# nnnagle/vq-vae

Measured on AMD Instinct MI355X. Metric: tiles/sec, higher is better.
Workload: dtype bf16

## Files before the change

vq-vae_amd/csrc/film_fused.hip:

```cpp
#include "frl_common.hpp"
#include "frl_host.hpp"
#include "frl_pack.hpp"
#include "frl_reduce.hpp"

typedef bf16x8 frag8;
#define FF_CZ 64
#define FF_HID 32
#define FF_C 12
#define FF_FR_W1 (4 * 2 * 64)
#define FF_FR_W2 64
#define FF_FR_W2T (2 * 64)
#define FF_FR_FWD (FF_FR_W1 + 2 * FF_FR_W2)
#define FF_FR_BWD (FF_FR_FWD + 2 * FF_FR_W2T)
#define FF_SLAB (2 * FF_HID * FF_CZ + 2 * FF_C * FF_HID + 2 * FF_HID + 2 * FF_C)

__device__ __forceinline__ void ff_pack_k4(frag8* __restrict__ dst, const float* __restrict__ W2, int tid, int nthreads) {
  for (int i = tid; i < FF_FR_W2T; i += nthreads) {
    const int lane = i & 63, mb = i >> 6;
    const int r = lane & 15, kc = lane >> 4;
    const int unit = 8 * (r >> 2) + 4 * mb + (r & 3);
    bf16x8 v;
#pragma unroll
    for (int e = 0; e < 8; ++e) {
      const int c = 4 * kc + e;
// ... 38 lines not shown
  }
  bool hit = false;
  frag8* pk = ws_pk;
  if (void* img = frl_pack_cached(jobs, n, off, &hit)) pk = (frag8*)img;
  if (!hit) FRL_LAUNCH(ff_pack_kernel, dim3(8), dim3(256), 0, st, pk, w1g, w1b, w2g, w2b, bwd);
  return pk;
}

__device__ __forceinline__ void ff_hidden(f32x4 (&ha)[4], const LQTile<bf16, 2>& zt, const frag8* __restrict__ w1, const float* __restrict__ tb,
                                          int lane, int kc) {
#pragma unroll
  for (int mb = 0; mb < 4; ++mb) {
    f32x4 acc = *reinterpret_cast<const f32x4*>(tb + 32 * (mb >> 1) + 8 * kc + 4 * (mb & 1));
    acc = mfma16(w1[(mb * 2 + 0) * 64 + lane], zt.f[0], acc);
    ha[mb] = mfma16(w1[(mb * 2 + 1) * 64 + lane], zt.f[1], acc);
  }
}
__device__ __forceinline__ frag8 ff_relu_frag(const f32x4& a, const f32x4& b) {
  return frag8{(bf16)fmaxf(a[0], 0.f), (bf16)fmaxf(a[1], 0.f), (bf16)fmaxf(a[2], 0.f), (bf16)fmaxf(a[3], 0.f),
               (bf16)fmaxf(b[0], 0.f), (bf16)fmaxf(b[1], 0.f), (bf16)fmaxf(b[2], 0.f), (bf16)fmaxf(b[3], 0.f)};
}

__device__ __forceinline__ void ff_tables(float* tb, const float* b1g, const float* b1b, const float* b2g, const float* b2b, int tid, int nthreads) {
  for (int i = tid; i < 96; i += nthreads) {
    float v = 0.f;
    if (i < 32) v = b1g[i];
    else if (i < 64) v = b1b[i - 32];
    else if (i < 80) v = (i - 64) < FF_C ? b2g[i - 64] : 0.f;
    else v = (i - 80) < FF_C ? b2b[i - 80] : 0.f;
    tb[i] = v;
  }
}

__global__ __launch_bounds__(256) void film_fused_fwd_kernel(const bf16* __restrict__ ZT, const bf16* __restrict__ Hh, const frag8* __restrict__ Wpk,
                                                             const float* __restrict__ b1g, const float* __restrict__ b1b,
                                                             const float* __restrict__ b2g, const float* __restrict__ b2b, bf16* __restrict__ Z,
                                                             bf16* __restrict__ GAM, bf16* __restrict__ BET, int64_t npix, int HW, int T) {
  extern __shared__ __attribute__((aligned(16))) char smem[];
  frag8* w1 = reinterpret_cast<frag8*>(smem);
  frag8* w2g = w1 + FF_FR_W1;
  frag8* w2b = w2g + FF_FR_W2;
  float* tb = reinterpret_cast<float*>(w2b + FF_FR_W2);
  const int tid = threadIdx.x, lane = tid & 63, wave = tid >> 6;
  const int px = lane & 15, kc = lane >> 4;
  copy_frags_lds<bf16>(w1, Wpk, FF_FR_FWD, tid, 256);
  ff_tables(tb, b1g, b1b, b2g, b2b, tid, 256);
  __syncthreads();
  const int64_t ntile = (npix + 15) >> 4;
  for (int64_t tile = (int64_t)blockIdx.x * 4 + wave; tile < ntile; tile += (int64_t)gridDim.x * 4) {
    const int64_t p = tile * 16 + px;
    const bool inb = p < npix;
    const int64_t pc = inb ? p : npix - 1;
    LQTile<bf16, 2> zt;
    lq_load<bf16, 2>(zt, ZT, pc, FF_CZ, kc, true);
    f32x4 ha[4];
    ff_hidden(ha, zt, w1, tb, lane, kc);
    const frag8 hg = ff_relu_frag(ha[0], ha[1]), hb = ff_relu_frag(ha[2], ha[3]);
    f32x4 g = mfma16(w2g[lane], hg, *reinterpret_cast<const f32x4*>(tb + 64 + 4 * kc));
    f32x4 bt = mfma16(w2b[lane], hb, *reinterpret_cast<const f32x4*>(tb + 80 + 4 * kc));
    if (!inb || kc == 3) continue;
    const bf16x4 gq = bf16x4{(bf16)g[0], (bf16)g[1], (bf16)g[2], (bf16)g[3]};
    const bf16x4 bq = bf16x4{(bf16)bt[0], (bf16)bt[1], (bf16)bt[2], (bf16)bt[3]};
    *reinterpret_cast<bf16x4*>(GAM + p * FF_C + 4 * kc) = gq;
    *reinterpret_cast<bf16x4*>(BET + p * FF_C + 4 * kc) = bq;
    const int64_t b = p / HW, hw = p - b * HW;
    const bf16* hp = Hh + ((b * T) * HW + hw) * FF_C + 4 * kc;
    bf16* zp = Z + ((b * T) * HW + hw) * FF_C + 4 * kc;
    for (int t = 0; t < T; ++t) {
      const bf16x4 hv = *reinterpret_cast<const bf16x4*>(hp + (int64_t)t * HW * FF_C);
      bf16x4 o;
#pragma unroll
      for (int e = 0; e < 4; ++e) o[e] = (bf16)fmaf((float)gq[e], (float)hv[e], (float)bq[e]);
      *reinterpret_cast<bf16x4*>(zp + (int64_t)t * HW * FF_C) = o;
    }
  }
}

#define FFB_R 64
#define FFB_P64 (64 + 8)
#define FFB_P32 (32 + 8)

__device__ __forceinline__ bf16x8 ff_tr_frag(const bf16* tile, int pitch, int pix0, int ch0, int r16) {
  const bf16* a0 = tile + (pix0 + (r16 >> 2)) * pitch + ch0 + 4 * (r16 & 3);
  bf16x4 lo = __builtin_amdgcn_ds_read_tr16_b64_v4bf16((bf16x4 __attribute__((address_space(3)))*)(a0));
  bf16x4 hi = __builtin_amdgcn_ds_read_tr16_b64_v4bf16((bf16x4 __attribute__((address_space(3)))*)(a0 + 4 * pitch));
  return bf16x8{lo[0], lo[1], lo[2], lo[3], hi[0], hi[1], hi[2], hi[3]};
}

__global__ __launch_bounds__(256) void film_fused_bwd_kernel(const bf16* __restrict__ ZT, const bf16* __restrict__ Hh, const bf16* __restrict__ DZ,
                                                             const frag8* __restrict__ Wpk, const float* __restrict__ b1g,
                                                             const float* __restrict__ b1b, const float* __restrict__ b2g,
                                                             const float* __restrict__ b2b, bf16* __restrict__ DH, float* __restrict__ slab,
                                                             int64_t npix, int HW, int T) {
  extern __shared__ __attribute__((aligned(16))) char smem[];
  frag8* w1 = reinterpret_cast<frag8*>(smem);
  frag8* w2g = w1 + FF_FR_W1;
  frag8* w2b = w2g + FF_FR_W2;
  frag8* w2gT = w2b + FF_FR_W2;
  frag8* w2bT = w2gT + FF_FR_W2T;
  float* tb = reinterpret_cast<float*>(w2bT + FF_FR_W2T);
  bf16* t_z = reinterpret_cast<bf16*>(tb + 96);
  bf16* t_hid = t_z + FFB_R * FFB_P64;
  bf16* t_dhid = t_hid + FFB_R * FFB_P64;
  bf16* t_dgb = t_dhid + FFB_R * FFB_P64;
  const int tid = threadIdx.x, lane = tid & 63, wave = tid >> 6;
  const int px = lane & 15, kc = lane >> 4, r16 = px;
  const int prow = wave * 16 + px;
  copy_frags_lds<bf16>(w1, Wpk, FF_FR_BWD, tid, 256);
  ff_tables(tb, b1g, b1b, b2g, b2b, tid, 256);
  __syncthreads();
  const bf16 one = (bf16)1.f, zero = (bf16)0.f;
  const bf16x8 ones = (r16 == 0) ? bf16x8{one, one, one, one, one, one, one, one} : bf16x8{zero, zero, zero, zero, zero, zero, zero, zero};
  const bf16x8 zeros = bf16x8{zero, zero, zero, zero, zero, zero, zero, zero};
  f32x4 gW1[4], gb1, gW2, gb2;
#pragma unroll
  for (int i = 0; i < 4; ++i) gW1[i] = f32x4{0.f, 0.f, 0.f, 0.f};
  gb1 = gW2 = gb2 = f32x4{0.f, 0.f, 0.f, 0.f};
  const int64_t nround = (npix + FFB_R - 1) / FFB_R;
  for (int64_t rd = blockIdx.x; rd < nround; rd += gridDim.x) {
    const int64_t p = rd * FFB_R + prow;
    const bool inb = p < npix;
    const int64_t pc = inb ? p : npix - 1;
    LQTile<bf16, 2> zt;
    lq_load<bf16, 2>(zt, ZT, pc, FF_CZ, kc, true);
    f32x4 ha[4];
    ff_hidden(ha, zt, w1, tb, lane, kc);
    const frag8 hg = ff_relu_frag(ha[0], ha[1]), hb = ff_relu_frag(ha[2], ha[3]);
    const f32x4 g = mfma16(w2g[lane], hg, *reinterpret_cast<const f32x4*>(tb + 64 + 4 * kc));
    float gq[4];
#pragma unroll
    for (int e = 0; e < 4; ++e) gq[e] = (float)(bf16)g[e];
    float dg[4] = {0.f, 0.f, 0.f, 0.f}, db[4] = {0.f, 0.f, 0.f, 0.f};
    if (inb && kc < 3) {
      const int64_t b = p / HW, hw = p - b * HW;
      const int64_t row0 = ((b * T) * HW + hw) * FF_C + 4 * kc;
      for (int t = 0; t < T; ++t) {
        const int64_t o = row0 + (int64_t)t * HW * FF_C;
        const bf16x4 dz = *reinterpret_cast<const bf16x4*>(DZ + o);
        const bf16x4 hv = *reinterpret_cast<const bf16x4*>(Hh + o);
        bf16x4 dh;
#pragma unroll
        for (int e = 0; e < 4; ++e) {
          const float d = (float)dz[e];
          dg[e] = fmaf(d, (float)hv[e], dg[e]);
          db[e] += d;
          dh[e] = (bf16)(gq[e] * d);
        }
        *reinterpret_cast<bf16x4*>(DH + o) = dh;
      }
    }
    const bf16x4 dgq = bf16x4{(bf16)dg[0], (bf16)dg[1], (bf16)dg[2], (bf16)dg[3]};
    const bf16x4 dbq = bf16x4{(bf16)db[0], (bf16)db[1], (bf16)db[2], (bf16)db[3]};
    const frag8 dgf = frag8{dgq[0], dgq[1], dgq[2], dgq[3], zero, zero, zero, zero};
    const frag8 dbf = frag8{dbq[0], dbq[1], dbq[2], dbq[3], zero, zero, zero, zero};
    f32x4 dha[4];
#pragma unroll
    for (int m = 0; m < 2; ++m) {
      dha[m] = mfma16(w2gT[m * 64 + lane], dgf, f32x4{0.f, 0.f, 0.f, 0.f});
      dha[2 + m] = mfma16(w2bT[m * 64 + lane], dbf, f32x4{0.f, 0.f, 0.f, 0.f});
    }
    frag8 dhf[2];
#pragma unroll
    for (int n = 0; n < 2; ++n)
#pragma unroll
      for (int e = 0; e < 8; ++e) dhf[n][e] = (bf16)(ha[2 * n + (e >> 2)][e & 3] > 0.f ? dha[2 * n + (e >> 2)][e & 3] : 0.f);
    {
      bf16x8* zp = reinterpret_cast<bf16x8*>(t_z + prow * FFB_P64 + 16 * kc);
      zp[0] = inb ? zt.f[0] : zeros;
      zp[1] = inb ? zt.f[1] : zeros;
      *reinterpret_cast<bf16x8*>(t_hid + prow * FFB_P64 + 8 * kc) = hg;
      *reinterpret_cast<bf16x8*>(t_hid + prow * FFB_P64 + 32 + 8 * kc) = hb;
      *reinterpret_cast<bf16x8*>(t_dhid + prow * FFB_P64 + 8 * kc) = dhf[0];
      *reinterpret_cast<bf16x8*>(t_dhid + prow * FFB_P64 + 32 + 8 * kc) = dhf[1];
      *reinterpret_cast<bf16x4*>(t_dgb + prow * FFB_P32 + 4 * kc) = dgq;
      *reinterpret_cast<bf16x4*>(t_dgb + prow * FFB_P32 + 16 + 4 * kc) = dbq;
    }
    __syncthreads();
#pragma unroll
    for (int ks = 0; ks < FFB_R / 32; ++ks) {
      const int pix0 = ks * 32 + 8 * kc;
      const bf16x8 ad = ff_tr_frag(t_dhid, FFB_P64, pix0, 16 * wave, r16);
#pragma unroll
      for (int i = 0; i < 4; ++i) gW1[i] = mfma16(ad, ff_tr_frag(t_z, FFB_P64, pix0, 16 * i, r16), gW1[i]);
      gb1 = mfma16(ad, ones, gb1);
      const bf16x8 ag = ff_tr_frag(t_dgb, FFB_P32, pix0, 16 * (wave >> 1), r16);
      gW2 = mfma16(ag, ff_tr_frag(t_hid, FFB_P64, pix0, 16 * wave, r16), gW2);
      if ((wave & 1) == 0) gb2 = mfma16(ag, ones, gb2);
    }
    __syncthreads();
  }
  float* my = slab + (int64_t)blockIdx.x * FF_SLAB;
  const int net = wave >> 1, row0 = 16 * (wave & 1);
#pragma unroll
  for (int i = 0; i < 4; ++i)
#pragma unroll
    for (int r = 0; r < 4; ++r) my[net * 2048 + (row0 + 4 * kc + r) * FF_CZ + 16 * i + r16] = gW1[i][r];
  if (r16 == 0) {
#pragma unroll
    for (int r = 0; r < 4; ++r) my[4864 + 32 * net + row0 + 4 * kc + r] = gb1[r];
  }
#pragma unroll
  for (int r = 0; r < 4; ++r) {
    const int c = 4 * kc + r;
    if (c < FF_C) {
      my[4096 + 384 * net + c * FF_HID + row0 + r16] = gW2[r];
      if (r16 == 0 && (wave & 1) == 0) my[4928 + 12 * net + c] = gb2[r];
    }
  }
}


extern "C" {

int frl_film_fused_supported(int cond_dim, int hidden, int target_dim, int dtype) {
  return (dtype == FRL_BF16 && cond_dim == FF_CZ && hidden == FF_HID && target_dim == FF_C) ? 1 : 0;
}

size_t frl_film_fused_workspace_bytes(void) { return (size_t)FF_FR_BWD * sizeof(frag8) + 256 + (size_t)768 * FF_SLAB * sizeof(float); }

int frl_film_fused_fwd(const void* z_type, const void* h, const float* w1g, const float* b1g, const float* w2g, const float* b2g, const float* w1b,
                       const float* b1b, const float* w2b, const float* b2b, void* z, void* gamma, void* beta, int B, int T, int HW, void* ws,
                       size_t ws_bytes, hipStream_t stream) {
  const int64_t npix = (int64_t)B * HW;
  if (npix <= 0 || T <= 0) return frl_fail(-2, "film_fused_fwd: empty input");
  if (ws_bytes < frl_film_fused_workspace_bytes()) return frl_fail(-4, "film_fused_fwd: workspace too small");
  const frag8* pk = ff_packed(w1g, w1b, w2g, w2b, 0, reinterpret_cast<frag8*>(ws), stream);
  int64_t g = ((npix + 15) / 16 + 3) / 4;
  if (g > 2048) g = 2048;
  const size_t lds = (size_t)FF_FR_FWD * sizeof(frag8) + 96 * sizeof(float);
  FRL_LAUNCH(film_fused_fwd_kernel, dim3((unsigned)g), dim3(256), lds, stream, (const bf16*)z_type, (const bf16*)h, pk, b1g, b1b, b2g, b2b, (bf16*)z,
             (bf16*)gamma, (bf16*)beta, npix, HW, T);
  return frl_check_launch("film_fused_fwd");
}

int frl_film_fused_bwd(const void* z_type, const void* h, const void* dz, const float* w1g, const float* b1g, const float* w2g, const float* b2g,
                       const float* w1b, const float* b1b, const float* w2b, const float* b2b, void* dh, float* dw1g, float* db1g, float* dw2g,
                       float* db2g, float* dw1b, float* db1b, float* dw2b, float* db2b, int B, int T, int HW, void* ws, size_t ws_bytes,
                       hipStream_t stream) {
  const int64_t npix = (int64_t)B * HW;
  if (npix <= 0 || T <= 0) return frl_fail(-2, "film_fused_bwd: empty input");
  if (ws_bytes < frl_film_fused_workspace_bytes()) return frl_fail(-4, "film_fused_bwd: workspace too small");
  char* w = (char*)ws;
  const size_t pkb = ((size_t)FF_FR_BWD * sizeof(frag8) + 255) / 256 * 256;
  const frag8* pk = ff_packed(w1g, w1b, w2g, w2b, 1, reinterpret_cast<frag8*>(w), stream);
  float* slab = reinterpret_cast<float*>(w + pkb);
  int64_t g = (npix + FFB_R - 1) / FFB_R;
  if (g > 768) g = 768;
  const size_t lds = (size_t)FF_FR_BWD * sizeof(frag8) + 96 * sizeof(float) + (size_t)FFB_R * (3 * FFB_P64 + FFB_P32) * sizeof(bf16);
  FRL_LAUNCH(film_fused_bwd_kernel, dim3((unsigned)g), dim3(256), lds, stream, (const bf16*)z_type, (const bf16*)h, (const bf16*)dz, pk, b1g, b1b, b2g,
             b2b, (bf16*)dh, slab, npix, HW, T);
  launch_slab_reduce_deferrable<float, FilmEpi>((const float*)slab, (int)g, (int64_t)FF_SLAB, FilmEpi{dw1g, dw1b, dw2g, dw2b, db1g, db1b, db2g, db2b}, stream);
  return frl_check_launch("film_fused_bwd");
}

}
```

vq-vae_amd/csrc/stencil.hip:

```cpp
#include "frl_common.hpp"
#include "frl_host.hpp"

#define ST_ND 4

__device__ __forceinline__ void st_dir(int i, int& dy, int& dx) {
  dy = (i == 0) ? 0 : 1;
  dx = (i == 0) ? 1 : (i == 1) ? 0 : (i == 2) ? 1 : -1;
}

template <typename T, int V>
__device__ __forceinline__ bool st_load(const T* __restrict__ X, int b, int y, int x, int H, int W, int C, int c0, float* v) {
  if (y < 0 || y >= H || x < 0 || x >= W) {
#pragma unroll
    for (int e = 0; e < V; ++e) v[e] = 0.f;
    return false;
  }
  Vec<T>::load(X + ((((int64_t)b * H + y) * W + x) * C + c0), v);
  return true;
}

struct StIdx { int b, y, x, c0; int64_t p; };
__device__ __forceinline__ StIdx st_index(int64_t i, int vpr, int V, int H, int W, bool small) {
  StIdx r;
  if (small) {
// ... 46 lines not shown
__global__ __launch_bounds__(256) void sobel_bwd_kernel(const T* __restrict__ DG, T* __restrict__ DX, const T* __restrict__ DXADD, int B, int H, int W,
                                                        int C) {
  const int vpr = C / V;
  const int64_t total = (int64_t)B * H * W * vpr;
  const bool small = total < ((int64_t)1 << 31);
  for (int64_t i = (int64_t)xcd_remap(blockIdx.x, gridDim.x) * 256 + threadIdx.x; i < total; i += (int64_t)gridDim.x * 256) {
    const StIdx ix = st_index(i, vpr, V, H, W, small);
    const int c0 = ix.c0, x = ix.x, y = ix.y, b = ix.b;
    const int64_t p = ix.p;
    float o[V];
    if (DXADD != nullptr) {
      Vec<T>::load(DXADD + p * C + c0, o);
    } else {
#pragma unroll
      for (int e = 0; e < V; ++e) o[e] = 0.f;
    }
#pragma unroll
    for (int ky = 0; ky < 3; ++ky)
#pragma unroll
      for (int kx = 0; kx < 3; ++kx) {
        if (ky == 1 && kx == 1) continue;
        const int qy = y - (ky - 1), qx = x - (kx - 1);
        if (qy < 0 || qy >= H || qx < 0 || qx >= W) continue;
        const float wx = (float)(kx - 1) * (ky == 1 ? 2.f : 1.f) * 0.25f;
        const float wy = (float)(ky - 1) * (kx == 1 ? 2.f : 1.f) * 0.25f;
        const int64_t qp = ((int64_t)b * H + qy) * W + qx;
        float a[V], c[V];
        Vec<T>::load(DG + qp * 2 * C + c0, a);
        Vec<T>::load(DG + qp * 2 * C + C + c0, c);
#pragma unroll
        for (int e = 0; e < V; ++e) o[e] = fmaf(wx, a[e], fmaf(wy, c[e], o[e]));
      }
    Vec<T>::store(DX + p * C + c0, o);
  }
}

template <typename T, int V, int R>
__global__ __launch_bounds__(256) void smooth_fwd_kernel(const T* __restrict__ X, const T* __restrict__ AL, const T* __restrict__ BL,
                                                         T* __restrict__ SM, T* __restrict__ RES, T* __restrict__ AS, T* __restrict__ BS,
                                                         int B, int H, int W, int C, int dil, int tpp) {
  constexpr int K = 2 * ST_ND;
  const int vpr = C / V;
  const int ppw = 256 / tpp;
  const int64_t npix = (int64_t)B * H * W;
  for (int64_t p = (int64_t)xcd_remap(blockIdx.x, gridDim.x) * ppw + threadIdx.x / tpp; p < npix; p += (int64_t)gridDim.x * ppw) {
    const int cvi = threadIdx.x % tpp;
    if (cvi >= vpr) continue;
    const int c0 = cvi * V;
    const int x = (int)(p % W), y = (int)((p / W) % H), b = (int)(p / ((int64_t)W * H));
    float A[K][R];
#pragma unroll
    for (int k = 0; k < K; ++k)
#pragma unroll
      for (int r = 0; r < R; ++r) A[k][r] = to_f32(AL[p * (K * R) + k * R + r]);
#pragma unroll
    for (int r = 0; r < R; ++r) {
      float m = A[0][r];
#pragma unroll
      for (int k = 1; k < K; ++k) m = fmaxf(m, A[k][r]);
      float s = 0.f;
#pragma unroll
      for (int k = 0; k < K; ++k) { A[k][r] = expf(A[k][r] - m); s += A[k][r]; }
      const float inv = 1.f / s;
#pragma unroll
      for (int k = 0; k < K; ++k) A[k][r] *= inv;
    }
// ... 447 lines not shown
                 (const bf16*)a3, (bf16*)o0, (bf16*)o1, (bf16*)o2, (const bf16*)o3, B, H, W, dil);
      return frl_check_launch("edge_smooth_stencil_bwd");
    }
  }
#define SM_CASE(RR)                                                                                                     \
  if (R == RR) {                                                                                                        \
    if (fwd) FRL_LAUNCH((smooth_fwd_kernel<T, V, RR>), dim3((unsigned)grid), dim3(256), 0, st, (const T*)a0, (const T*)a1, \
                                (const T*)a2, (T*)o0, (T*)o1, (T*)o2, (T*)o3, B, H, W, C, dil, tpp);                     \
    else FRL_LAUNCH((smooth_bwd_kernel<T, V, RR>), dim3((unsigned)grid), dim3(256), 0, st, (const T*)a0, (const T*)a1,      \
                            (const T*)a2, (const T*)a3, (T*)o0, (T*)o1, (T*)o2, (const T*)o3, B, H, W, C, dil, tpp);    \
    return frl_check_launch("edge_smooth_stencil");                                                                     \
  }
  SM_CASE(1) SM_CASE(2) SM_CASE(4)
#undef SM_CASE
  return frl_fail(-2, "edge_smooth: rank must be 1, 2 or 4");
}

extern "C" {

int frl_sobel_fwd(const void* x, void* g, int B, int H, int W, int C, int dtype, hipStream_t stream) {
  if (dtype == FRL_F32 && C % 4 == 0)
    FRL_LAUNCH((sobel_fwd_kernel<float, 4>), dim3(st_grid((int64_t)B * H * W * (C / 4))), dim3(256), 0, stream, (const float*)x, (float*)g, B, H, W, C);
  else if (dtype == FRL_BF16 && C % 8 == 0)
    FRL_LAUNCH((sobel_fwd_kernel<bf16, 8>), dim3(st_grid((int64_t)B * H * W * (C / 8))), dim3(256), 0, stream, (const bf16*)x, (bf16*)g, B, H, W, C);
  else return frl_fail(-2, "sobel: C must be a multiple of 8 (bf16) / 4 (f32)");
  return frl_check_launch("sobel_fwd");
}

static int sobel_bwd_launch(const void* dg, void* dx, const void* dx_add, int B, int H, int W, int C, int dtype, hipStream_t stream) {
  if (dtype == FRL_F32 && C % 4 == 0)
    FRL_LAUNCH((sobel_bwd_kernel<float, 4>), dim3(st_grid((int64_t)B * H * W * (C / 4))), dim3(256), 0, stream, (const float*)dg, (float*)dx,
               (const float*)dx_add, B, H, W, C);
  else if (dtype == FRL_BF16 && C % 8 == 0)
    FRL_LAUNCH((sobel_bwd_kernel<bf16, 8>), dim3(st_grid((int64_t)B * H * W * (C / 8))), dim3(256), 0, stream, (const bf16*)dg, (bf16*)dx,
               (const bf16*)dx_add, B, H, W, C);
  else return frl_fail(-2, "sobel: C must be a multiple of 8 (bf16) / 4 (f32)");
  return frl_check_launch("sobel_bwd");
}

int frl_sobel_bwd(const void* dg, void* dx, int B, int H, int W, int C, int dtype, hipStream_t stream) {
  return sobel_bwd_launch(dg, dx, nullptr, B, H, W, C, dtype, stream);
}

int frl_sobel_bwd_add(const void* dg, void* dx, const void* dx_add, int B, int H, int W, int C, int dtype, hipStream_t stream) {
  return sobel_bwd_launch(dg, dx, dx_add, B, H, W, C, dtype, stream);
}

int frl_edge_smooth_stencil_fwd(const void* x, const void* a_logit, const void* b_logit, void* smoothed, void* residual, void* a_soft,
                                void* b_soft, int B, int H, int W, int C, int R, int coarse_dilation, int dtype, hipStream_t stream) {
  if (dtype == FRL_F32 && C % 4 == 0)
    return smooth_dispatch<float, 4>(true, x, a_logit, b_logit, nullptr, smoothed, residual, a_soft, b_soft, B, H, W, C, R, coarse_dilation, stream);
  if (dtype == FRL_BF16 && C % 8 == 0)
    return smooth_dispatch<bf16, 8>(true, x, a_logit, b_logit, nullptr, smoothed, residual, a_soft, b_soft, B, H, W, C, R, coarse_dilation, stream);
  return frl_fail(-2, "edge_smooth: C must be a multiple of 8 (bf16) / 4 (f32)");
}

int frl_edge_smooth_stencil_bwd(const void* d_smoothed, const void* x, const void* a_soft, const void* b_soft, void* dx, void* da_logit,
                                void* db_logit, const void* dx_add, int B, int H, int W, int C, int R, int coarse_dilation, int dtype,
                                hipStream_t stream) {
  void* add = const_cast<void*>(dx_add);
  if (dtype == FRL_F32 && C % 4 == 0)
    return smooth_dispatch<float, 4>(false, d_smoothed, x, a_soft, b_soft, dx, da_logit, db_logit, add, B, H, W, C, R, coarse_dilation, stream);
  if (dtype == FRL_BF16 && C % 8 == 0)
    return smooth_dispatch<bf16, 8>(false, d_smoothed, x, a_soft, b_soft, dx, da_logit, db_logit, add, B, H, W, C, R, coarse_dilation, stream);
  return frl_fail(-2, "edge_smooth: C must be a multiple of 8 (bf16) / 4 (f32)");
}

}
// ... 1 lines not shown
```

vq-vae_amd/csrc/vq_bwd.hpp:

```cpp
#pragma once
#include "vq_common.hpp"

template <typename T>
__global__ __launch_bounds__(256) void vq_bwd_kernel(const T* __restrict__ gout, const T* __restrict__ Z,
                                                     const float* __restrict__ E, const int32_t* __restrict__ idx,
                                                     const float* __restrict__ gscale, float cz_base, int64_t N, int K, int d,
                                                     int Kc, int64_t rows_per_wg, T* __restrict__ gz,
                                                     float* __restrict__ slab ) {
  extern __shared__ __attribute__((aligned(16))) char smem[];
  float* acc = reinterpret_cast<float*>(smem);
  const int tid = threadIdx.x;
  const int64_t r0 = (int64_t)blockIdx.x * rows_per_wg;
  int64_t r1 = r0 + rows_per_wg;
  if (r1 > N) r1 = N;
  const float cz = cz_base * (gscale ? gscale[0] : 1.f);
  constexpr int VEC = DT<T>::VEC;
  const bool fast = (d % VEC) == 0;
  const int vpr = (d + VEC - 1) / VEC;
  const int nchunks = (K + Kc - 1) / Kc;
  for (int c = 0; c < nchunks; ++c) {
    const int kbase = c * Kc;
    __syncthreads();
    for (int i = tid; i < Kc * d; i += 256) acc[i] = 0.f;
    __syncthreads();
    const int64_t nvec = (r1 > r0 ? (r1 - r0) : 0) * vpr;
    for (int64_t i = tid; i < nvec; i += 256) {
      const int64_t n = r0 + i / vpr;
      const int c0 = (int)(i % vpr) * VEC;
      const int k = idx[n];
      const bool mine = (k >= kbase && k < kbase + Kc);
      if (c == 0 || mine) {
        float zv[VEC];
        if (fast) Vec<T>::load(Z + n * (int64_t)d + c0, zv);
        else {
// ... 15 lines not shown
            }
          } else {
#pragma unroll
            for (int e = 0; e < VEC; ++e) gv[e] = 0.f;
          }
#pragma unroll
          for (int e = 0; e < VEC; ++e) {
            const float ev = (c0 + e < d) ? to_f32(from_f32<T>(E[(int64_t)k * d + c0 + e])) : 0.f;
            ov[e] = gv[e] + cz * (zv[e] - ev);
          }
          if (fast) Vec<T>::store(gz + n * (int64_t)d + c0, ov);
          else {
#pragma unroll
            for (int e = 0; e < VEC; ++e)
              if (c0 + e < d) gz[n * (int64_t)d + c0 + e] = from_f32<T>(ov[e]);
          }
        }
      }
    }
    __syncthreads();
    const int kn = (K - kbase) < Kc ? (K - kbase) : Kc;
    float* dst = slab + ((int64_t)blockIdx.x * K + kbase) * d;
    for (int i = tid; i < kn * d; i += 256) dst[i] = acc[i];
  }
}

template <int RB, int CB, int NWV>
__global__ __launch_bounds__(64 * NWV) void vq_bwd_mfma_kernel(const bf16* __restrict__ gout, const bf16* __restrict__ Z, const bf16* __restrict__ ZQ,
                                                          const float* __restrict__ E,
                                                          const int32_t* __restrict__ idx, const float* __restrict__ gscale, float cz_base,
                                                          int64_t N, int K, int d, int64_t rows_per_wg, bf16* __restrict__ gz,
                                                          float* __restrict__ slab ) {
  constexpr int DP = CB * 16, PITCH = DP + 8, KC = RB * NWV * 16, NTH = 64 * NWV;
  extern __shared__ __attribute__((aligned(16))) char smem[];
  bf16* zt = reinterpret_cast<bf16*>(smem);
  int* it = reinterpret_cast<int*>(zt + 64 * PITCH);
  const int tid = threadIdx.x, lane = tid & 63, wave = tid >> 6;
  const int r16 = lane & 15, kc = lane >> 4;
  const int64_t r0 = (int64_t)blockIdx.x * rows_per_wg;
  int64_t r1 = r0 + rows_per_wg;
  if (r1 > N) r1 = N;
  const float cz = cz_base * (gscale ? gscale[0] : 1.f);
  const bool fast = (d % 8) == 0;
  const int vpr = DP / 8;
  const bf16 one = (bf16)1.f, zero = (bf16)0.f;
  for (int kbase = 0; kbase < K; kbase += KC) {
    f32x4 acc[RB][CB];
#pragma unroll
    for (int a = 0; a < RB; ++a)
#pragma unroll
      for (int b = 0; b < CB; ++b) acc[a][b] = f32x4{0.f, 0.f, 0.f, 0.f};
    constexpr int NV = (64 * (DP / 8) + NTH - 1) / NTH;
    const bool pre = fast && (ZQ != nullptr || gz == nullptr || kbase != 0);
    const bool want_gz = (kbase == 0 && gz != nullptr);
    bf16x8 rz[NV], rg[NV], rq[NV];
    auto fetch = [&](int64_t p0) {
#pragma unroll
      for (int u = 0; u < NV; ++u) {
        const int i = tid + u * NTH;
        const int row = i / vpr, c0 = (i % vpr) * 8;
        const int64_t n = p0 + row;
        const bool ok = i < 64 * vpr && n < r1 && c0 < d;
        const int64_t off = ok ? n * (int64_t)d + c0 : 0;
        bf16x8 v = *reinterpret_cast<const bf16x8*>(Z + off);
        if (!ok) v = bf16x8{};
        rz[u] = v;
        if (want_gz) {
          rg[u] = gout != nullptr ? *reinterpret_cast<const bf16x8*>(gout + off) : bf16x8{};
          rq[u] = *reinterpret_cast<const bf16x8*>(ZQ + off);
        }
      }
    };
    if (pre && r0 < r1) fetch(r0);
    for (int64_t p0 = r0; p0 < r1; p0 += 64) {
      __syncthreads();
      if (pre) {
#pragma unroll
        for (int u = 0; u < NV; ++u) {
          const int i = tid + u * NTH;
          if (i >= 64 * vpr) continue;
          const int row = i / vpr, c0 = (i % vpr) * 8;
          const int64_t n = p0 + row;
          if (want_gz && n < r1 && c0 < d) {
            float ov[8];
#pragma unroll
            for (int e = 0; e < 8; ++e) ov[e] = (float)rg[u][e] + cz * ((float)rz[u][e] - (float)rq[u][e]);
            Vec<bf16>::store(gz + n * (int64_t)d + c0, ov);
          }
          *reinterpret_cast<bf16x8*>(zt + row * PITCH + c0) = rz[u];
        }
      } else {
      for (int i = tid; i < 64 * vpr; i += NTH) {
        const int row = i / vpr, c0 = (i % vpr) * 8;
        const int64_t n = p0 + row;
        float zv[8];
#pragma unroll
        for (int e = 0; e < 8; ++e) zv[e] = 0.f;
        if (n < r1 && c0 < d) {
          if (fast) Vec<bf16>::load(Z + n * (int64_t)d + c0, zv);
          else {
#pragma unroll
            for (int e = 0; e < 8; ++e) if (c0 + e < d) zv[e] = (float)Z[n * (int64_t)d + c0 + e];
          }
          if (kbase == 0 && gz != nullptr) {
            const int k = idx[n];
            float gv[8], ov[8];
#pragma unroll
            for (int e = 0; e < 8; ++e) gv[e] = 0.f;
            if (gout != nullptr) {
              if (fast) Vec<bf16>::load(gout + n * (int64_t)d + c0, gv);
              else {
#pragma unroll
                for (int e = 0; e < 8; ++e) if (c0 + e < d) gv[e] = (float)gout[n * (int64_t)d + c0 + e];
              }
            }
            float qv[8];
            if (ZQ != nullptr && fast) Vec<bf16>::load(ZQ + n * (int64_t)d + c0, qv);
            else {
#pragma unroll
              for (int e = 0; e < 8; ++e) qv[e] = (c0 + e < d) ? (float)(bf16)E[(int64_t)k * d + c0 + e] : 0.f;
            }
#pragma unroll
            for (int e = 0; e < 8; ++e) ov[e] = gv[e] + cz * (zv[e] - qv[e]);
            if (fast) Vec<bf16>::store(gz + n * (int64_t)d + c0, ov);
            else {
#pragma unroll
              for (int e = 0; e < 8; ++e) if (c0 + e < d) gz[n * (int64_t)d + c0 + e] = (bf16)ov[e];
            }
          }
        }
        Vec<bf16>::store(zt + row * PITCH + c0, zv);
      }
      }
      if (tid < 64) it[tid] = (p0 + tid < r1) ? idx[p0 + tid] - kbase : -1;
      __syncthreads();
      if (pre && p0 + 64 < r1) fetch(p0 + 64);
#pragma unroll
      for (int ks = 0; ks < 2; ++ks) {
        const int pix0 = ks * 32 + 8 * kc;
        int id8[8];
#pragma unroll
        for (int j = 0; j < 8; ++j) id8[j] = it[pix0 + j];
        bf16x8 bfr[CB];
#pragma unroll
        for (int b = 0; b < CB; ++b) {
          const bf16* a0 = zt + (pix0 + (r16 >> 2)) * PITCH + b * 16 + 4 * (r16 & 3);
          bf16x4 lo = __builtin_amdgcn_ds_read_tr16_b64_v4bf16((bf16x4 __attribute__((address_space(3)))*)(a0));
          bf16x4 hi = __builtin_amdgcn_ds_read_tr16_b64_v4bf16((bf16x4 __attribute__((address_space(3)))*)(a0 + 4 * PITCH));
          bfr[b] = bf16x8{lo[0], lo[1], lo[2], lo[3], hi[0], hi[1], hi[2], hi[3]};
        }
#pragma unroll
        for (int a = 0; a < RB; ++a) {
          const int code = (wave * RB + a) * 16 + r16;
          bf16x8 af;
#pragma unroll
          for (int j = 0; j < 8; ++j) af[j] = (id8[j] == code) ? one : zero;
#pragma unroll
          for (int b = 0; b < CB; ++b) acc[a][b] = mfma16(af, bfr[b], acc[a][b]);
        }
      }
    }
    float* dst = slab + (int64_t)blockIdx.x * K * d;
#pragma unroll
    for (int a = 0; a < RB; ++a)
#pragma unroll
      for (int b = 0; b < CB; ++b)
#pragma unroll
        for (int r = 0; r < 4; ++r) {
          const int k = kbase + (wave * RB + a) * 16 + kc * 4 + r, c = b * 16 + r16;
          if (k < K && c < d) dst[(int64_t)k * d + c] = acc[a][b][r];
        }
  }
}

template <typename T>
__global__ void vq_code_reduce_kernel(const float* __restrict__ slab, int nslab, const float* __restrict__ E,
                                      const int32_t* __restrict__ counts, const float* __restrict__ gscale, float ce_base,
                                      int K, int d, float* __restrict__ gE, float* __restrict__ sums_out) {
  const int64_t i = (int64_t)blockIdx.x * blockDim.x + threadIdx.x;
  if (i >= (int64_t)K * d) return;
  float s = 0.f;
  for (int w = 0; w < nslab; ++w) s += slab[(int64_t)w * K * d + i];
  if (sums_out) sums_out[i] = s;
  if (gE) {
    const float ce = ce_base * (gscale ? gscale[1] : 1.f);
    const float ev = to_f32(from_f32<T>(E[i]));
    gE[i] = ce * ((float)counts[i / d] * ev - s);
  }
}

__global__ __launch_bounds__(256) void vq_ema_kernel(const float* __restrict__ sums, const int32_t* __restrict__ counts, int K, int d,
                                                     float decay, float eps, float* __restrict__ ema_count,
                                                     float* __restrict__ ema_sum, float* __restrict__ E, const float* __restrict__ ok) {
// ... 42 lines not shown
```

Measured before the change: 109,700.

## Software-pipeline FiLM fwd/bwd loads, add sobel strip kernel, ring-buffer VQ bwd fetch

The FiLM forward and backward kernels now double-buffer their per-tile loads, issuing the next tile's ZT and H/DZ reads before the current tile's compute. They also specialise on T==5 so the time loop fully unrolls into register arrays, and the forward grid cap drops to 768 workgroups. A new bf16 sobel backward strip kernel computes two output rows per thread and reuses the loaded neighbour rows. The VQ backward kernel switches to a three-deep register ring of nontemporal prefetches when RB=CB=4. Together these aim to hide global memory latency and cut redundant loads, at the cost of higher register pressure and more code paths.

Measured after the change: 109,400. About the same (-0.3%).

```diff
diff --git a/vq-vae_amd/csrc/film_fused.hip b/vq-vae_amd/csrc/film_fused.hip
--- a/vq-vae_amd/csrc/film_fused.hip
+++ b/vq-vae_amd/csrc/film_fused.hip
@@ -94,6 +94,30 @@
   }
 }
 
+__device__ __forceinline__ int64_t ff_row0(int64_t p, int HW, int T) {
+  const int64_t b = (p >> 31) == 0 ? (int64_t)((unsigned)p / (unsigned)HW) : p / HW;
+  return (p + b * (int64_t)(T - 1) * HW) * FF_C;
+}
+
+#define FF_FWD_WGS 768
+template <int TC> struct FfRowsF {
+  LQTile<bf16, 2> zt;
+  bf16x4 hv[TC > 0 ? TC : 1];
+  int64_t row0;
+};
+template <int TC>
+__device__ __forceinline__ void ff_request_fwd(FfRowsF<TC>& r, const bf16* __restrict__ ZT, const bf16* __restrict__ Hh, int64_t tile, int px, int kc,
+                                               int64_t npix, int HW, int T) {
+  const int64_t p = tile * 16 + px, pc = p < npix ? p : npix - 1;
+  lq_load<bf16, 2>(r.zt, ZT, pc, FF_CZ, kc, true);
+  r.row0 = ff_row0(pc, HW, T) + 4 * (kc < 3 ? kc : 2);
+  if constexpr (TC > 0) {
+#pragma unroll
+    for (int t = 0; t < TC; ++t) r.hv[t] = *reinterpret_cast<const bf16x4*>(Hh + r.row0 + (int64_t)t * HW * FF_C);
+  }
+}
+
+template <int TC>
 __global__ __launch_bounds__(256) void film_fused_fwd_kernel(const bf16* __restrict__ ZT, const bf16* __restrict__ Hh, const frag8* __restrict__ Wpk,
                                                              const float* __restrict__ b1g, const float* __restrict__ b1b,
                                                              const float* __restrict__ b2g, const float* __restrict__ b2b, bf16* __restrict__ Z,
@@ -105,36 +129,55 @@
   float* tb = reinterpret_cast<float*>(w2b + FF_FR_W2);
   const int tid = threadIdx.x, lane = tid & 63, wave = tid >> 6;
   const int px = lane & 15, kc = lane >> 4;
+  const int64_t ntile = (npix + 15) >> 4, tstep = (int64_t)gridDim.x * 4;
+  int64_t tile = (int64_t)blockIdx.x * 4 + wave;
+  FfRowsF<TC> ra, rb;
+  ff_request_fwd<TC>(ra, ZT, Hh, tile < ntile ? tile : ntile - 1, px, kc, npix, HW, T);
   copy_frags_lds<bf16>(w1, Wpk, FF_FR_FWD, tid, 256);
   ff_tables(tb, b1g, b1b, b2g, b2b, tid, 256);
   __syncthreads();
-  const int64_t ntile = (npix + 15) >> 4;
-  for (int64_t tile = (int64_t)blockIdx.x * 4 + wave; tile < ntile; tile += (int64_t)gridDim.x * 4) {
-    const int64_t p = tile * 16 + px;
-    const bool inb = p < npix;
-    const int64_t pc = inb ? p : npix - 1;
-    LQTile<bf16, 2> zt;
-    lq_load<bf16, 2>(zt, ZT, pc, FF_CZ, kc, true);
+  auto tile_out = [&](const FfRowsF<TC>& r, int64_t tl) {
+    const int64_t p = tl * 16 + px;
     f32x4 ha[4];
-    ff_hidden(ha, zt, w1, tb, lane, kc);
+    ff_hidden(ha, r.zt, w1, tb, lane, kc);
     const frag8 hg = ff_relu_frag(ha[0], ha[1]), hb = ff_relu_frag(ha[2], ha[3]);
     f32x4 g = mfma16(w2g[lane], hg, *reinterpret_cast<const f32x4*>(tb + 64 + 4 * kc));
     f32x4 bt = mfma16(w2b[lane], hb, *reinterpret_cast<const f32x4*>(tb + 80 + 4 * kc));
-    if (!inb || kc == 3) continue;
-    const bf16x4 gq = bf16x4{(bf16)g[0], (bf16)g[1], (bf16)g[2], (bf16)g[3]};
-    const bf16x4 bq = bf16x4{(bf16)bt[0], (bf16)bt[1], (bf16)bt[2], (bf16)bt[3]};
-    *reinterpret_cast<bf16x4*>(GAM + p * FF_C + 4 * kc) = gq;
-    *reinterpret_cast<bf16x4*>(BET + p * FF_C + 4 * kc) = bq;
-    const int64_t b = p / HW, hw = p - b * HW;
-    const bf16* hp = Hh + ((b * T) * HW + hw) * FF_C + 4 * kc;
-    bf16* zp = Z + ((b * T) * HW + hw) * FF_C + 4 * kc;
-    for (int t = 0; t < T; ++t) {
-      const bf16x4 hv = *reinterpret_cast<const bf16x4*>(hp + (int64_t)t * HW * FF_C);
-      bf16x4 o;
-#pragma unroll
-      for (int e = 0; e < 4; ++e) o[e] = (bf16)fmaf((float)gq[e], (float)hv[e], (float)bq[e]);
-      *reinterpret_cast<bf16x4*>(zp + (int64_t)t * HW * FF_C) = o;
-    }
+    if (p < npix && kc < 3) {
+      const bf16x4 gq = bf16x4{(bf16)g[0], (bf16)g[1], (bf16)g[2], (bf16)g[3]};
+      const bf16x4 bq = bf16x4{(bf16)bt[0], (bf16)bt[1], (bf16)bt[2], (bf16)bt[3]};
+      *reinterpret_cast<bf16x4*>(GAM + p * FF_C + 4 * kc) = gq;
+      *reinterpret_cast<bf16x4*>(BET + p * FF_C + 4 * kc) = bq;
+      bf16* zp = Z + r.row0;
+      if constexpr (TC > 0) {
+#pragma unroll
+        for (int t = 0; t < TC; ++t) {
+          bf16x4 o;
+#pragma unroll
+          for (int e = 0; e < 4; ++e) o[e] = (bf16)fmaf((float)gq[e], (float)r.hv[t][e], (float)bq[e]);
+          *reinterpret_cast<bf16x4*>(zp + (int64_t)t * HW * FF_C) = o;
+        }
+      } else {
+        const bf16* hp = Hh + r.row0;
+        for (int t = 0; t < T; ++t) {
+          const bf16x4 hv = *reinterpret_cast<const bf16x4*>(hp + (int64_t)t * HW * FF_C);
+          bf16x4 o;
+#pragma unroll
+          for (int e = 0; e < 4; ++e) o[e] = (bf16)fmaf((float)gq[e], (float)hv[e], (float)bq[e]);
+          *reinterpret_cast<bf16x4*>(zp + (int64_t)t * HW * FF_C) = o;
+        }
+      }
+    }
+  };
+  while (tile < ntile) {
+    const int64_t t1 = tile + tstep;
+    ff_request_fwd<TC>(rb, ZT, Hh, t1 < ntile ? t1 : tile, px, kc, npix, HW, T);
+    tile_out(ra, tile);
+    if (t1 >= ntile) break;
+    const int64_t t2 = t1 + tstep;
+    ff_request_fwd<TC>(ra, ZT, Hh, t2 < ntile ? t2 : t1, px, kc, npix, HW, T);
+    tile_out(rb, t1);
+    tile = t2;
   }
 }
 
@@ -149,7 +192,29 @@
   return bf16x8{lo[0], lo[1], lo[2], lo[3], hi[0], hi[1], hi[2], hi[3]};
 }
 
-__global__ __launch_bounds__(256) void film_fused_bwd_kernel(const bf16* __restrict__ ZT, const bf16* __restrict__ Hh, const bf16* __restrict__ DZ,
+template <int TC> struct FfRowsB {
+  LQTile<bf16, 2> zt;
+  bf16x4 dz[TC > 0 ? TC : 1], hv[TC > 0 ? TC : 1];
+  int64_t row0;
+};
+template <int TC>
+__device__ __forceinline__ void ff_request_bwd(FfRowsB<TC>& r, const bf16* __restrict__ ZT, const bf16* __restrict__ Hh, const bf16* __restrict__ DZ,
+                                               int64_t p, int kc, int64_t npix, int HW, int T) {
+  const int64_t pc = p < npix ? p : npix - 1;
+  lq_load<bf16, 2>(r.zt, ZT, pc, FF_CZ, kc, true);
+  r.row0 = ff_row0(pc, HW, T) + 4 * (kc < 3 ? kc : 2);
+  if constexpr (TC > 0) {
+#pragma unroll
+    for (int t = 0; t < TC; ++t) {
+      const int64_t o = r.row0 + (int64_t)t * HW * FF_C;
+      r.dz[t] = __builtin_nontemporal_load(reinterpret_cast<const bf16x4*>(DZ + o));
+      r.hv[t] = __builtin_nontemporal_load(reinterpret_cast<const bf16x4*>(Hh + o));
+    }
+  }
+}
+
+template <int TC>
+__global__ __launch_bounds__(256, 3) void film_fused_bwd_kernel(const bf16* __restrict__ ZT, const bf16* __restrict__ Hh, const bf16* __restrict__ DZ,
                                                              const frag8* __restrict__ Wpk, const float* __restrict__ b1g,
                                                              const float* __restrict__ b1b, const float* __restrict__ b2g,
                                                              const float* __restrict__ b2b, bf16* __restrict__ DH, float* __restrict__ slab,
@@ -168,6 +233,10 @@
   const int tid = threadIdx.x, lane = tid & 63, wave = tid >> 6;
   const int px = lane & 15, kc = lane >> 4, r16 = px;
   const int prow = wave * 16 + px;
+  const int64_t nround = (npix + FFB_R - 1) / FFB_R;
+  const int64_t rstep = gridDim.x;
+  FfRowsB<TC> ra, rb;
+  ff_request_bwd<TC>(ra, ZT, Hh, DZ, ((int64_t)blockIdx.x < nround ? (int64_t)blockIdx.x : nround - 1) * FFB_R + prow, kc, npix, HW, T);
   copy_frags_lds<bf16>(w1, Wpk, FF_FR_BWD, tid, 256);
   ff_tables(tb, b1g, b1b, b2g, b2b, tid, 256);
   __syncthreads();
@@ -178,13 +247,10 @@
 #pragma unroll
   for (int i = 0; i < 4; ++i) gW1[i] = f32x4{0.f, 0.f, 0.f, 0.f};
   gb1 = gW2 = gb2 = f32x4{0.f, 0.f, 0.f, 0.f};
-  const int64_t nround = (npix + FFB_R - 1) / FFB_R;
-  for (int64_t rd = blockIdx.x; rd < nround; rd += gridDim.x) {
+  auto do_round = [&](const FfRowsB<TC>& cur, int64_t rd, FfRowsB<TC>& nxt, int64_t rn) {
     const int64_t p = rd * FFB_R + prow;
     const bool inb = p < npix;
-    const int64_t pc = inb ? p : npix - 1;
-    LQTile<bf16, 2> zt;
-    lq_load<bf16, 2>(zt, ZT, pc, FF_CZ, kc, true);
+    const LQTile<bf16, 2>& zt = cur.zt;
     f32x4 ha[4];
     ff_hidden(ha, zt, w1, tb, lane, kc);
     const frag8 hg = ff_relu_frag(ha[0], ha[1]), hb = ff_relu_frag(ha[2], ha[3]);
@@ -194,23 +260,39 @@
     for (int e = 0; e < 4; ++e) gq[e] = (float)(bf16)g[e];
     float dg[4] = {0.f, 0.f, 0.f, 0.f}, db[4] = {0.f, 0.f, 0.f, 0.f};
     if (inb && kc < 3) {
-      const int64_t b = p / HW, hw = p - b * HW;
-      const int64_t row0 = ((b * T) * HW + hw) * FF_C + 4 * kc;
-      for (int t = 0; t < T; ++t) {
-        const int64_t o = row0 + (int64_t)t * HW * FF_C;
-        const bf16x4 dz = *reinterpret_cast<const bf16x4*>(DZ + o);
-        const bf16x4 hv = *reinterpret_cast<const bf16x4*>(Hh + o);
-        bf16x4 dh;
-#pragma unroll
-        for (int e = 0; e < 4; ++e) {
-          const float d = (float)dz[e];
-          dg[e] = fmaf(d, (float)hv[e], dg[e]);
-          db[e] += d;
-          dh[e] = (bf16)(gq[e] * d);
+      const int64_t row0 = cur.row0;
+      if constexpr (TC > 0) {
+#pragma unroll
+        for (int t = 0; t < TC; ++t) {
+          const int64_t o = row0 + (int64_t)t * HW * FF_C;
+          bf16x4 dh;
+#pragma unroll
+          for (int e = 0; e < 4; ++e) {
+            const float d = (float)cur.dz[t][e];
+            dg[e] = fmaf(d, (float)cur.hv[t][e], dg[e]);
+            db[e] += d;
+            dh[e] = (bf16)(gq[e] * d);
+          }
+          *reinterpret_cast<bf16x4*>(DH + o) = dh;
         }
-        *reinterpret_cast<bf16x4*>(DH + o) = dh;
+      } else {
+        for (int t = 0; t < T; ++t) {
+          const int64_t o = row0 + (int64_t)t * HW * FF_C;
+          const bf16x4 dz = *reinterpret_cast<const bf16x4*>(DZ + o);
+          const bf16x4 hv = *reinterpret_cast<const bf16x4*>(Hh + o);
+          bf16x4 dh;
+#pragma unroll
+          for (int e = 0; e < 4; ++e) {
+            const float d = (float)dz[e];
+            dg[e] = fmaf(d, (float)hv[e], dg[e]);
+            db[e] += d;
+            dh[e] = (bf16)(gq[e] * d);
+          }
+          *reinterpret_cast<bf16x4*>(DH + o) = dh;
+        }
       }
     }
+    ff_request_bwd<TC>(nxt, ZT, Hh, DZ, rn * FFB_R + prow, kc, npix, HW, T);
     const bf16x4 dgq = bf16x4{(bf16)dg[0], (bf16)dg[1], (bf16)dg[2], (bf16)dg[3]};
     const bf16x4 dbq = bf16x4{(bf16)db[0], (bf16)db[1], (bf16)db[2], (bf16)db[3]};
     const frag8 dgf = frag8{dgq[0], dgq[1], dgq[2], dgq[3], zero, zero, zero, zero};
@@ -250,6 +332,14 @@
       if ((wave & 1) == 0) gb2 = mfma16(ag, ones, gb2);
     }
     __syncthreads();
+  };
+  for (int64_t rd = blockIdx.x; rd < nround;) {
+    const int64_t r1 = rd + rstep;
+    do_round(ra, rd, rb, r1 < nround ? r1 : rd);
+    if (r1 >= nround) break;
+    const int64_t r2 = r1 + rstep;
+    do_round(rb, r1, ra, r2 < nround ? r2 : r1);
+    rd = r2;
   }
   float* my = slab + (int64_t)blockIdx.x * FF_SLAB;
   const int net = wave >> 1, row0 = 16 * (wave & 1);
@@ -288,10 +378,14 @@
   if (ws_bytes < frl_film_fused_workspace_bytes()) return frl_fail(-4, "film_fused_fwd: workspace too small");
   const frag8* pk = ff_packed(w1g, w1b, w2g, w2b, 0, reinterpret_cast<frag8*>(ws), stream);
   int64_t g = ((npix + 15) / 16 + 3) / 4;
-  if (g > 2048) g = 2048;
+  if (g > FF_FWD_WGS) g = FF_FWD_WGS;
   const size_t lds = (size_t)FF_FR_FWD * sizeof(frag8) + 96 * sizeof(float);
-  FRL_LAUNCH(film_fused_fwd_kernel, dim3((unsigned)g), dim3(256), lds, stream, (const bf16*)z_type, (const bf16*)h, pk, b1g, b1b, b2g, b2b, (bf16*)z,
-             (bf16*)gamma, (bf16*)beta, npix, HW, T);
+  if (T == 5)
+    FRL_LAUNCH(film_fused_fwd_kernel<5>, dim3((unsigned)g), dim3(256), lds, stream, (const bf16*)z_type, (const bf16*)h, pk, b1g, b1b, b2g, b2b,
+               (bf16*)z, (bf16*)gamma, (bf16*)beta, npix, HW, T);
+  else
+    FRL_LAUNCH(film_fused_fwd_kernel<0>, dim3((unsigned)g), dim3(256), lds, stream, (const bf16*)z_type, (const bf16*)h, pk, b1g, b1b, b2g, b2b,
+               (bf16*)z, (bf16*)gamma, (bf16*)beta, npix, HW, T);
   return frl_check_launch("film_fused_fwd");
 }
 
@@ -309,8 +403,12 @@
   int64_t g = (npix + FFB_R - 1) / FFB_R;
   if (g > 768) g = 768;
   const size_t lds = (size_t)FF_FR_BWD * sizeof(frag8) + 96 * sizeof(float) + (size_t)FFB_R * (3 * FFB_P64 + FFB_P32) * sizeof(bf16);
-  FRL_LAUNCH(film_fused_bwd_kernel, dim3((unsigned)g), dim3(256), lds, stream, (const bf16*)z_type, (const bf16*)h, (const bf16*)dz, pk, b1g, b1b, b2g,
-             b2b, (bf16*)dh, slab, npix, HW, T);
+  if (T == 5)
+    FRL_LAUNCH(film_fused_bwd_kernel<5>, dim3((unsigned)g), dim3(256), lds, stream, (const bf16*)z_type, (const bf16*)h, (const bf16*)dz, pk, b1g, b1b,
+               b2g, b2b, (bf16*)dh, slab, npix, HW, T);
+  else
+    FRL_LAUNCH(film_fused_bwd_kernel<0>, dim3((unsigned)g), dim3(256), lds, stream, (const bf16*)z_type, (const bf16*)h, (const bf16*)dz, pk, b1g, b1b,
+               b2g, b2b, (bf16*)dh, slab, npix, HW, T);
   launch_slab_reduce_deferrable<float, FilmEpi>((const float*)slab, (int)g, (int64_t)FF_SLAB, FilmEpi{dw1g, dw1b, dw2g, dw2b, db1g, db1b, db2g, db2b}, stream);
   return frl_check_launch("film_fused_bwd");
 }
diff --git a/vq-vae_amd/csrc/stencil.hip b/vq-vae_amd/csrc/stencil.hip
--- a/vq-vae_amd/csrc/stencil.hip
+++ b/vq-vae_amd/csrc/stencil.hip
@@ -102,6 +102,68 @@
         for (int e = 0; e < V; ++e) o[e] = fmaf(wx, a[e], fmaf(wy, c[e], o[e]));
       }
     Vec<T>::store(DX + p * C + c0, o);
+  }
+}
+
+#define ST_SOBEL_ROWS 2
+template <int SR, bool ADD>
+__global__ __launch_bounds__(256) void sobel_bwd_strip_kernel(const bf16* __restrict__ DG, bf16* __restrict__ DX, const bf16* __restrict__ DXADD, int B,
+                                                              int H, int W, int C) {
+  constexpr int V = 8;
+  const int vpr = C / V;
+  const int SH = (H + SR - 1) / SR;
+  const int64_t total = (int64_t)B * SH * W * vpr;
+  const bool small = total < ((int64_t)1 << 31);
+  for (int64_t i = (int64_t)xcd_remap(blockIdx.x, gridDim.x) * 256 + threadIdx.x; i < total; i += (int64_t)gridDim.x * 256) {
+    const StIdx ix = st_index(i, vpr, V, SH, W, small);
+    const int c0 = ix.c0, x = ix.x, y0 = ix.y * SR, b = ix.b;
+    bf16x8 ga[SR + 2][3], gc[SR + 2][3];
+    const bool okx[3] = {x > 0, true, x + 1 < W};
+#pragma unroll
+    for (int j = 0; j < SR + 2; ++j) {
+      const int qy = y0 - 1 + j, qyc = qy < 0 ? 0 : (qy < H ? qy : H - 1);
+#pragma unroll
+      for (int k = 0; k < 3; ++k) {
+        const int qxc = okx[k] ? x - 1 + k : x;
+        const bf16* q = DG + ((((int64_t)b * H + qyc) * W + qxc) * 2 * C + c0);
+        ga[j][k] = *reinterpret_cast<const bf16x8*>(q);
+        gc[j][k] = *reinterpret_cast<const bf16x8*>(q + C);
+      }
+    }
+    bf16x8 ad[ADD ? SR : 1];
+    if constexpr (ADD) {
+#pragma unroll
+      for (int r = 0; r < SR; ++r) {
+        const int yc = y0 + r < H ? y0 + r : H - 1;
+        ad[r] = *reinterpret_cast<const bf16x8*>(DXADD + ((((int64_t)b * H + yc) * W + x) * C + c0));
+      }
+    }
+#pragma unroll
+    for (int r = 0; r < SR; ++r) {
+      const int y = y0 + r;
+      if (y >= H) break;
+      float o[V];
+      if constexpr (ADD) {
+#pragma unroll
+        for (int e = 0; e < V; ++e) o[e] = (float)ad[r][e];
+      } else {
+#pragma unroll
+        for (int e = 0; e < V; ++e) o[e] = 0.f;
+      }
+#pragma unroll
+      for (int ky = 0; ky < 3; ++ky)
+#pragma unroll
+        for (int kx = 0; kx < 3; ++kx) {
+          if (ky == 1 && kx == 1) continue;
+          const int qy = y - (ky - 1), j = r + 2 - ky, k = 2 - kx;
+          if (qy < 0 || qy >= H || !okx[k]) continue;
+          const float wx = (float)(kx - 1) * (ky == 1 ? 2.f : 1.f) * 0.25f;
+          const float wy = (float)(ky - 1) * (kx == 1 ? 2.f : 1.f) * 0.25f;
+#pragma unroll
+          for (int e = 0; e < V; ++e) o[e] = fmaf(wx, (float)ga[j][k][e], fmaf(wy, (float)gc[j][k][e], o[e]));
+        }
+      Vec<bf16>::store(DX + ((((int64_t)b * H + y) * W + x) * C + c0), o);
+    }
   }
 }
 
@@ -615,8 +677,13 @@
     FRL_LAUNCH((sobel_bwd_kernel<float, 4>), dim3(st_grid((int64_t)B * H * W * (C / 4))), dim3(256), 0, stream, (const float*)dg, (float*)dx,
                (const float*)dx_add, B, H, W, C);
   else if (dtype == FRL_BF16 && C % 8 == 0)
-    FRL_LAUNCH((sobel_bwd_kernel<bf16, 8>), dim3(st_grid((int64_t)B * H * W * (C / 8))), dim3(256), 0, stream, (const bf16*)dg, (bf16*)dx,
-               (const bf16*)dx_add, B, H, W, C);
+  {
+    const dim3 grid(st_grid((int64_t)B * ((H + ST_SOBEL_ROWS - 1) / ST_SOBEL_ROWS) * W * (C / 8)));
+    if (dx_add != nullptr)
+      FRL_LAUNCH((sobel_bwd_strip_kernel<ST_SOBEL_ROWS, true>), grid, dim3(256), 0, stream, (const bf16*)dg, (bf16*)dx, (const bf16*)dx_add, B, H, W, C);
+    else
+      FRL_LAUNCH((sobel_bwd_strip_kernel<ST_SOBEL_ROWS, false>), grid, dim3(256), 0, stream, (const bf16*)dg, (bf16*)dx, (const bf16*)dx_add, B, H, W, C);
+  }
   else return frl_fail(-2, "sobel: C must be a multiple of 8 (bf16) / 4 (f32)");
   return frl_check_launch("sobel_bwd");
 }
diff --git a/vq-vae_amd/csrc/vq_bwd.hpp b/vq-vae_amd/csrc/vq_bwd.hpp
--- a/vq-vae_amd/csrc/vq_bwd.hpp
+++ b/vq-vae_amd/csrc/vq_bwd.hpp
@@ -1,5 +1,6 @@
 #pragma once
 #include "vq_common.hpp"
+#include <type_traits>
 
 template <typename T>
 __global__ __launch_bounds__(256) void vq_bwd_kernel(const T* __restrict__ gout, const T* __restrict__ Z,
@@ -81,6 +82,7 @@
                                                           int64_t N, int K, int d, int64_t rows_per_wg, bf16* __restrict__ gz,
                                                           float* __restrict__ slab ) {
   constexpr int DP = CB * 16, PITCH = DP + 8, KC = RB * NWV * 16, NTH = 64 * NWV;
+  constexpr int VQB_RING = (RB == 4 && CB == 4) ? 3 : 1;
   extern __shared__ __attribute__((aligned(16))) char smem[];
   bf16* zt = reinterpret_cast<bf16*>(smem);
   int* it = reinterpret_cast<int*>(zt + 64 * PITCH);
@@ -102,43 +104,94 @@
     constexpr int NV = (64 * (DP / 8) + NTH - 1) / NTH;
     const bool pre = fast && (ZQ != nullptr || gz == nullptr || kbase != 0);
     const bool want_gz = (kbase == 0 && gz != nullptr);
-    bf16x8 rz[NV], rg[NV], rq[NV];
-    auto fetch = [&](int64_t p0) {
+    bf16x8 rz[VQB_RING][NV], rg[VQB_RING][NV], rq[VQB_RING][NV];
+    int ri[VQB_RING];
+    const bf16* gsrc = gout != nullptr ? gout : Z;
+    auto fetch = [&](auto with_gz, bf16x8 (&fz)[NV], bf16x8 (&fg)[NV], bf16x8 (&fq)[NV], int& fi, int64_t p0) {
 #pragma unroll
       for (int u = 0; u < NV; ++u) {
         const int i = tid + u * NTH;
         const int row = i / vpr, c0 = (i % vpr) * 8;
-        const int64_t n = p0 + row;
-        const bool ok = i < 64 * vpr && n < r1 && c0 < d;
-        const int64_t off = ok ? n * (int64_t)d + c0 : 0;
-        bf16x8 v = *reinterpret_cast<const bf16x8*>(Z + off);
-        if (!ok) v = bf16x8{};
-        rz[u] = v;
-        if (want_gz) {
-          rg[u] = gout != nullptr ? *reinterpret_cast<const bf16x8*>(gout + off) : bf16x8{};
-          rq[u] = *reinterpret_cast<const bf16x8*>(ZQ + off);
-        }
-      }
+        const int64_t n = p0 + row < r1 ? p0 + row : r1 - 1;
+        const int64_t off = n * (int64_t)d + (c0 < d ? c0 : 0);
+        fz[u] = __builtin_nontemporal_load(reinterpret_cast<const bf16x8*>(Z + off));
+        if constexpr (decltype(with_gz)::value) {
+          fg[u] = __builtin_nontemporal_load(reinterpret_cast<const bf16x8*>(gsrc + off));
+          fq[u] = __builtin_nontemporal_load(reinterpret_cast<const bf16x8*>(ZQ + off));
+        }
+      }
+      const int64_t ni = p0 + lane < r1 ? p0 + lane : r1 - 1;
+      fi = idx[ni];
     };
-    if (pre && r0 < r1) fetch(r0);
+    auto contract = [&]() {
+#pragma unroll
+    for (int ks = 0; ks < 2; ++ks) {
+      const int pix0 = ks * 32 + 8 * kc;
+      int id8[8];
+#pragma unroll
+      for (int j = 0; j < 8; ++j) id8[j] = it[pix0 + j];
+      bf16x8 bfr[CB];
+#pragma unroll
+      for (int b = 0; b < CB; ++b) {
+        const bf16* a0 = zt + (pix0 + (r16 >> 2)) * PITCH + b * 16 + 4 * (r16 & 3);
+        bf16x4 lo = __builtin_amdgcn_ds_read_tr16_b64_v4bf16((bf16x4 __attribute__((address_space(3)))*)(a0));
+        bf16x4 hi = __builtin_amdgcn_ds_read_tr16_b64_v4bf16((bf16x4 __attribute__((address_space(3)))*)(a0 + 4 * PITCH));
+        bfr[b] = bf16x8{lo[0], lo[1], lo[2], lo[3], hi[0], hi[1], hi[2], hi[3]};
+      }
+#pragma unroll
+      for (int a = 0; a < RB; ++a) {
+        const int code = (wave * RB + a) * 16 + r16;
+        bf16x8 af;
+#pragma unroll
+        for (int j = 0; j < 8; ++j) af[j] = (id8[j] == code) ? one : zero;
+#pragma unroll
+        for (int b = 0; b < CB; ++b) acc[a][b] = mfma16(af, bfr[b], acc[a][b]);
+      }
+    }
+    };
+    auto ring = [&](auto with_gz) {
+      constexpr bool WG = decltype(with_gz)::value;
+#pragma unroll
+      for (int s = 0; s < VQB_RING; ++s) fetch(with_gz, rz[s], rg[s], rq[s], ri[s], r0 + 64 * s);
+      for (int64_t pb = r0; pb < r1; pb += 64 * VQB_RING) {
+#pragma unroll
+        for (int s = 0; s < VQB_RING; ++s) {
+          const int64_t p0 = pb + 64 * s;
+          if (p0 >= r1) break;
+          __syncthreads();
+#pragma unroll
+          for (int u = 0; u < NV; ++u) {
+            const int i = tid + u * NTH;
+            if (i >= 64 * vpr) continue;
+            const int row = i / vpr, c0 = (i % vpr) * 8;
+            const int64_t n = p0 + row;
+            const bool ok = n < r1 && c0 < d;
+            if constexpr (WG) {
+              if (ok) {
+                float ov[8];
+#pragma unroll
+                for (int e = 0; e < 8; ++e)
+                  ov[e] = (gout != nullptr ? (float)rg[s][u][e] : 0.f) + cz * ((float)rz[s][u][e] - (float)rq[s][u][e]);
+                Vec<bf16>::store(gz + n * (int64_t)d + c0, ov);
+              }
+            }
+            *reinterpret_cast<bf16x8*>(zt + row * PITCH + c0) = ok ? rz[s][u] : bf16x8{};
+          }
+          if (tid < 64) it[tid] = (p0 + tid < r1) ? ri[s] - kbase : -1;
+          __syncthreads();
+          fetch(with_gz, rz[s], rg[s], rq[s], ri[s], p0 + 64 * VQB_RING);
+          contract();
+        }
+      }
+    };
+    if (pre) {
+      if (r0 < r1) {
+        if (want_gz) ring(std::true_type{});
+        else ring(std::false_type{});
+      }
+    } else {
     for (int64_t p0 = r0; p0 < r1; p0 += 64) {
       __syncthreads();
-      if (pre) {
-#pragma unroll
-        for (int u = 0; u < NV; ++u) {
-          const int i = tid + u * NTH;
-          if (i >= 64 * vpr) continue;
-          const int row = i / vpr, c0 = (i % vpr) * 8;
-          const int64_t n = p0 + row;
-          if (want_gz && n < r1 && c0 < d) {
-            float ov[8];
-#pragma unroll
-            for (int e = 0; e < 8; ++e) ov[e] = (float)rg[u][e] + cz * ((float)rz[u][e] - (float)rq[u][e]);
-            Vec<bf16>::store(gz + n * (int64_t)d + c0, ov);
-          }
-          *reinterpret_cast<bf16x8*>(zt + row * PITCH + c0) = rz[u];
-        }
-      } else {
       for (int i = tid; i < 64 * vpr; i += NTH) {
         const int row = i / vpr, c0 = (i % vpr) * 8;
         const int64_t n = p0 + row;
@@ -180,34 +233,10 @@
         }
         Vec<bf16>::store(zt + row * PITCH + c0, zv);
       }
-      }
       if (tid < 64) it[tid] = (p0 + tid < r1) ? idx[p0 + tid] - kbase : -1;
       __syncthreads();
-      if (pre && p0 + 64 < r1) fetch(p0 + 64);
-#pragma unroll
-      for (int ks = 0; ks < 2; ++ks) {
-        const int pix0 = ks * 32 + 8 * kc;
-        int id8[8];
-#pragma unroll
-        for (int j = 0; j < 8; ++j) id8[j] = it[pix0 + j];
-        bf16x8 bfr[CB];
-#pragma unroll
-        for (int b = 0; b < CB; ++b) {
-          const bf16* a0 = zt + (pix0 + (r16 >> 2)) * PITCH + b * 16 + 4 * (r16 & 3);
-          bf16x4 lo = __builtin_amdgcn_ds_read_tr16_b64_v4bf16((bf16x4 __attribute__((address_space(3)))*)(a0));
-          bf16x4 hi = __builtin_amdgcn_ds_read_tr16_b64_v4bf16((bf16x4 __attribute__((address_space(3)))*)(a0 + 4 * PITCH));
-          bfr[b] = bf16x8{lo[0], lo[1], lo[2], lo[3], hi[0], hi[1], hi[2], hi[3]};
-        }
-#pragma unroll
-        for (int a = 0; a < RB; ++a) {
-          const int code = (wave * RB + a) * 16 + r16;
-          bf16x8 af;
-#pragma unroll
-          for (int j = 0; j < 8; ++j) af[j] = (id8[j] == code) ? one : zero;
-#pragma unroll
-          for (int b = 0; b < CB; ++b) acc[a][b] = mfma16(af, bfr[b], acc[a][b]);
-        }
-      }
+      contract();
+    }
     }
     float* dst = slab + (int64_t)blockIdx.x * K * d;
 #pragma unroll
```
